# zouyuoz/SVS-UNet-PyTorch

Measured on AMD Instinct MI355X. Metric: spectrogram-tiles/sec (512x128) U-Net fwd+bwd (L1 train step incl. Adam), higher is better.
Workload: dtype f32; 1 GPU; train.py L1-loss step, 512x128 tiles, batch 64 per GPU; global_batch=64, parallelism=dp1, mode=train

## Files before the change

svs_unet_pytorch_amd/csrc/common.h:

```cpp
#pragma once
#include <hip/hip_runtime.h>
#include <stdint.h>
#include <stdio.h>
#include <string>

#include "../../include/svs_hip.h"

typedef float f32x4 __attribute__((ext_vector_type(4)));

void svs_set_error(const char* fmt, ...);

#define SVS_REQUIRE(cond, ...)                 \
  do {                                         \
    if (!(cond)) {                             \
      svs_set_error(__VA_ARGS__);              \
      return SVS_ERR_INVALID;                  \
    }                                          \
  } while (0)

#define SVS_CHECK_LAUNCH(name)                                                     \
  do {                                                                             \
    hipError_t e_ = hipGetLastError();                                             \
    if (e_ != hipSuccess) {                                                        \
      svs_set_error("%s: launch failed: %s", name, hipGetErrorString(e_));         \
      return (int)e_;                                                              \
    }                                                                              \
  } while (0)

#define SVS_HIP(call)                                                              \
  do {                                                                             \
    hipError_t e_ = (call);                                                        \
    if (e_ != hipSuccess) {                                                        \
      svs_set_error("%s failed: %s", #call, hipGetErrorString(e_));                \
      return (int)e_;                                                              \
    }                                                                              \
  } while (0)

static inline bool svs_aligned16(const void* p) { return (((uintptr_t)p) & 15u) == 0; }
static inline int svs_cdiv(long a, long b) { return (int)((a + b - 1) / b); }
static inline size_t svs_align_up(size_t x, size_t a) { return (x + a - 1) / a * a; }

enum SvsTune {
  SVS_TUNE_CONV_CFG, SVS_TUNE_CONV_KSPLIT, SVS_TUNE_CONV_WINDOW, SVS_TUNE_CONV_SKIP, SVS_TUNE_SKIP_REDUCE,
  SVS_TUNE_WGRAD_CFG, SVS_TUNE_WGRAD_KSPLIT, SVS_TUNE_WGRAD_SKIP, SVS_TUNE_WGRAD_WINDOW, SVS_TUNE_TRAIN_UNFUSED,
  SVS_TUNE_TRAIN_ONE_STREAM, SVS_TUNE_MFMA_SPLIT, SVS_TUNE_CONV_C1_TILED, SVS_TUNE_BF16_CFG, SVS_TUNE_BF16_KSPLIT,
  SVS_TUNE_BN_INLINE, SVS_TUNE_CONV_GWINDOW, SVS_TUNE_COUNT
};
long svs_tune(int key);
static inline bool svs_tune_on(int key) { return svs_tune(key) >= 0; }
static inline bool svs_tune_flag(int key) { return svs_tune(key) > 0; }

static inline int svs_conv_out(int n) { return (n + 1) / 2; }

__device__ __forceinline__ float svs_wave_sum(float v) {
#pragma unroll
  for (int o = 32; o > 0; o >>= 1) v += __shfl_xor(v, o, 64);
  return v;
}

__host__ __device__ __forceinline__ uint32_t svs_mix32(uint32_t x) {
  x ^= x >> 16; x *= 0x7FEB352Du; x ^= x >> 15; x *= 0x846CA68Bu; x ^= x >> 16;
  return x;
}
__host__ __device__ __forceinline__ uint32_t svs_u32(uint32_t seed, uint64_t idx) {
  uint32_t lo = (uint32_t)idx, hi = (uint32_t)(idx >> 32);
  uint32_t s = svs_mix32(seed + 1u);
  uint32_t h = svs_mix32(hi + 0x85EBCA6Bu * s);
  return svs_mix32(lo + 0x9E3779B9u * h);
}
```

svs_unet_pytorch_amd/csrc/gemm_wgrad.hip:

```cpp
#include <stdlib.h>

#include "internal.h"
#include "mfma_split.h"

struct WgradArgs {
  const float* s; long lds; int Hs, Ws, Cs;
  const float* l; long ldl; int Hl, Wl, Cl;
  int B;
  float* slab;
  long pix_per_split;
  int ws_shift, hs_shift;
  int b_shift;
};

template <int T> __device__ __forceinline__ void load_vec(const float* p, float (&f)[T]);
template <> __device__ __forceinline__ void load_vec<4>(const float* p, float (&f)[4]) {
  const f32x4 v = *(const f32x4*)p; f[0] = v[0]; f[1] = v[1]; f[2] = v[2]; f[3] = v[3];
}
template <> __device__ __forceinline__ void load_vec<2>(const float* p, float (&f)[2]) {
  const float2 v = *(const float2*)p; f[0] = v.x; f[1] = v.y;
}
template <int T> __device__ __forceinline__ void store_vec(float* p, const float (&f)[T]);
template <> __device__ __forceinline__ void store_vec<4>(float* p, const float (&f)[4]) { *(f32x4*)p = (f32x4){f[0], f[1], f[2], f[3]}; }
template <> __device__ __forceinline__ void store_vec<2>(float* p, const float (&f)[2]) { *(float2*)p = make_float2(f[0], f[1]); }
// ... 300 lines not shown
    }
  };
  auto stage = [&]() {
#pragma unroll
    for (int r = 0; r < RS; ++r) {
      const int e = t + 256 * r;
      if (e < NS) *(f32x4*)(&Ssm[(e / (CSB / 4)) * LS + (e % (CSB / 4)) * 4]) = sreg[r];
    }
#pragma unroll
    for (int r = 0; r < RL; ++r) {
      const int e = t + 256 * r;
      if (e < NL) *(f32x4*)(&Lsm[(e >> 2) * LL + (e & 3) * 4]) = lreg[r];
    }
  };

  f32x4 acc[25];
#pragma unroll
  for (int i = 0; i < 25; ++i) acc[i] = (f32x4){0.f, 0.f, 0.f, 0.f};
  const float* abase = &Ssm[(half * (TH / KS) * TW + q) * LS + mt * 16 + lrow];
  const float* bbase = &Lsm[(half * (TH / KS) * 2 * LW + 2 * q) * LL + lrow];

  if (tile_lo < tile_hi) fetch(tile_lo);
  for (int tile = tile_lo; tile < tile_hi; ++tile) {
    __syncthreads();
    stage();
    __syncthreads();
    if (tile + 1 < tile_hi) fetch(tile + 1);
#pragma unroll
    for (int ks = 0; ks < KSTEPS; ++ks) {
      const int sh = ks / 4, sg = ks % 4;
      const float a = abase[(sh * TW + sg * 4) * LS];
#pragma unroll
      for (int tap = 0; tap < 25; ++tap) {
        const int kh = tap / 5, kw = tap % 5;
        const float bv = bbase[((2 * sh + kh) * LW + 8 * sg + kw) * LL];
        acc[tap] = __builtin_amdgcn_mfma_f32_16x16x4f32(a, bv, acc[tap], 0, 0, 0);
      }
    }
  }
  const int Ntot = 25 * p.Cl;
  float* slab = p.slab + ((long)blockIdx.x * KS + half) * p.Cs * Ntot;
#pragma unroll
  for (int tap = 0; tap < 25; ++tap)
#pragma unroll
    for (int r = 0; r < 4; ++r)
      slab[(long)(m0 + mt * 16 + 4 * q + r) * Ntot + tap * p.Cl + cl0 + lrow] = acc[tap][r];
}

__global__ __launch_bounds__(256) void wgrad_reduce_kernel(const float* __restrict__ slab, int ksplit, int Cs, int Cl,
                                                           float* __restrict__ dw) {
  __shared__ float tile[25][65];
  const int clt = Cl < 64 ? Cl : 64;
  const int cs = blockIdx.x, cl0 = blockIdx.y * clt;
  const long zstride = (long)Cs * Cl * 25;
  const float* src0 = slab + (long)cs * 25 * Cl + cl0;
  const int q4 = clt >> 2;
  for (int e = threadIdx.x; e < 25 * q4; e += 256) {
    const int tap = e / q4, cl = (e - tap * q4) * 4;
    const float* src = src0 + (long)tap * Cl + cl;
    f32x4 acc = {0.f, 0.f, 0.f, 0.f};
    int z = 0;
    for (; z + 4 <= ksplit; z += 4, src += 4 * zstride) {
      const f32x4 a = *(const f32x4*)src, b = *(const f32x4*)(src + zstride), c = *(const f32x4*)(src + 2 * zstride), d = *(const f32x4*)(src + 3 * zstride);
      acc += a; acc += b; acc += c; acc += d;
    }
    for (; z < ksplit; ++z, src += zstride) acc += *(const f32x4*)src;
    tile[tap][cl] = acc[0]; tile[tap][cl + 1] = acc[1]; tile[tap][cl + 2] = acc[2]; tile[tap][cl + 3] = acc[3];
  }
  __syncthreads();
  float* dst = dw + ((long)cs * Cl + cl0) * 25;
  for (int e = threadIdx.x; e < 25 * clt; e += 256) {
    const int cl = e / 25, tap = e - cl * 25;
    dst[e] = tile[tap][cl];
  }
}

struct WgradTile { int cfg, BM, BN, ksplit; long pps; };
static WgradTile plan_wgrad(int B, int Hs, int Ws, int Cs, int Cl) {
  WgradTile pl{};
  if (Cs % 128 == 0) { pl.cfg = 0; pl.BM = 128; }
  else if (Cs % 64 == 0) { pl.cfg = 1; pl.BM = 64; }
  else { pl.cfg = 2; pl.BM = 32; }
  if (pl.cfg == 0 && ((long)B * Hs * Ws <= 1024 || Cl <= 32)) { pl.cfg = 1; pl.BM = 64; }
  if (svs_tune_on(SVS_TUNE_WGRAD_CFG)) {
    const int c = (int)svs_tune(SVS_TUNE_WGRAD_CFG);
    if (c == 0 && Cs % 128 == 0) { pl.cfg = 0; pl.BM = 128; }
    if (c == 1 && Cs % 64 == 0) { pl.cfg = 1; pl.BM = 64; }
    if (c == 2 && Cs % 32 == 0) { pl.cfg = 2; pl.BM = 32; }
  }
  pl.BN = 128;
  const long P = (long)B * Hs * Ws;
  const long blocks_mn = (long)(Cs / pl.BM) * ((25L * Cl + pl.BN - 1) / pl.BN);
  long ks = (1024 + blocks_mn - 1) / blocks_mn;
  const long cap = P / 128 > 1 ? P / 128 : 1;
  if (ks > cap) ks = cap;
  if (ks > 512) ks = 512;
  if (ks < 1) ks = 1;
  if (svs_tune_on(SVS_TUNE_WGRAD_KSPLIT)) { long f = svs_tune(SVS_TUNE_WGRAD_KSPLIT); if (f >= 1 && f <= cap) ks = f; }
  long pps = (P + ks - 1) / ks;
  pps = (pps + 15) / 16 * 16;
  ks = (P + pps - 1) / pps;
  pl.ksplit = (int)ks;
  pl.pps = pps;
  return pl;
}

#define WG_GROUPS 8

struct WgWinPlan { int eligible, use, MT, gy, gx, tpb, ntiles, nslab; };
static WgWinPlan plan_wgrad_window(int B, int Hs, int Ws, int Cs, int Cl) {
  WgWinPlan w{};
  w.eligible = (Cl == 16 || Cl == 32) && (Cs == 32 || Cs == 64 || Cs == 128);
  w.ntiles = B * ((Hs + 3) / 4) * ((Ws + 15) / 16);
  w.use = w.eligible && w.ntiles >= 1024;
  if (svs_tune_on(SVS_TUNE_WGRAD_WINDOW)) { const int f = (int)svs_tune(SVS_TUNE_WGRAD_WINDOW); w.use = (f == 0) ? 0 : (f == 2) ? w.eligible : w.use; }
  if (!w.eligible) return w;
  w.MT = (Cs % 64 == 0) ? 4 : 2;
  w.gy = (Cs / (16 * w.MT)) * (Cl / 16);
  int gx = 512 / w.gy;
  if (gx > w.ntiles) gx = w.ntiles;
  w.tpb = (w.ntiles + gx - 1) / gx;
  w.gx = (w.ntiles + w.tpb - 1) / w.tpb;
  w.nslab = w.gx * (4 / w.MT);
  return w;
}

struct WgradPlan {
  WgWinPlan win;
  WgradTile tile;
  int WM, WN, pf;
  bool skip, split;
  dim3 grid;
  int nslab;
};
static WgradPlan plan_wgrad_call(int B, int Hs, int Ws, int Cs, int Cl, long lds, int Hl, int Wl, long ldl) {
  WgradPlan p{};
  p.win = plan_wgrad_window(B, Hs, Ws, Cs, Cl);
  p.win.use = p.win.use && (long)Hs * Ws * lds * 4 < (1L << 31) && (long)Hl * Wl * ldl * 4 < (1L << 31);
  if (p.win.use) {
    p.grid = dim3(p.win.gx, p.win.gy);
    p.nslab = p.win.nslab;
    return p;
  }
  p.tile = plan_wgrad(B, Hs, Ws, Cs, Cl);
  p.WM = p.tile.cfg == 0 ? 2 : 1;
  p.WN = 4 / p.WM;
  const bool can_skip = B >= 16 && (B & (B - 1)) == 0 && (Ws & (Ws - 1)) == 0 && (long)B * Hs * Ws * lds * 4 < (1L << 31);
  const long f = svs_tune(SVS_TUNE_WGRAD_SKIP);
  p.skip = f == 0 ? false : f == 2 ? can_skip : can_skip && Ws <= 8;
  p.pf = p.skip && p.tile.cfg <= 1 ? 2 : 1;
  p.split = svs_tune(SVS_TUNE_MFMA_SPLIT) > 0;
  p.grid = dim3((unsigned)(Cs / p.tile.BM), (unsigned)((25 * Cl + p.tile.BN - 1) / p.tile.BN), (unsigned)p.tile.ksplit);
  p.nslab = p.tile.ksplit;
  return p;
}

size_t svs_wgrad_gemm_workspace(int B, int Hs, int Ws, int Cs, int Cl) {
  const WgWinPlan w = plan_wgrad_window(B, Hs, Ws, Cs, Cl);
  int nslab = plan_wgrad(B, Hs, Ws, Cs, Cl).ksplit;
  if (w.eligible && w.nslab > nslab) nslab = w.nslab;
  return ((size_t)nslab + WG_GROUPS) * Cs * 25 * Cl * sizeof(float);
}

static int wgrad_reduce_run(const float* slabs, int nslab, int Cs, int Cl, float* dw, float* tmp, hipStream_t stream) {
  const long n = (long)Cs * 25 * Cl;
  if (nslab > 2 * WG_GROUPS) {
    const int per = (nslab + WG_GROUPS - 1) / WG_GROUPS;
    const int groups = (nslab + per - 1) / per;
    if (int rc = svs_reduce_slabs_run(slabs, nslab, per, groups, n, tmp, stream)) return rc;
    slabs = tmp;
    nslab = groups;
  }
// ... 67 lines not shown
```

svs_unet_pytorch_amd/csrc/internal.h:

```cpp
#pragma once
#include "common.h"

enum { SVS_MODE_GATHER = 0, SVS_MODE_PARITY = 1 };

int svs_conv_gemm_run(int mode, const float* x, long ldx, int B, int H, int W, int C, const float* wp,
                      const float* bias, const float* scale, const float* shift, float slope, float* y, long ldy,
                      int Ho, int Wo, int N, int accumulate, void* ws, size_t ws_bytes, hipStream_t stream,
                      const char* who, float* stats = nullptr, int stats_cap = 0, int* stats_nblk = nullptr);
int svs_bn_finalize_run(const void* partial, int nblk, long P, int C, float eps, float momentum, float* running_mean,
                        float* running_var, long long* nbt, float* save_mean, float* save_invstd, hipStream_t stream);
int svs_bn_fin_act_apply_run(const void* partial, int rows, const float* raw, long ldr, long P, int C, long pixels_per_sample,
                             const float* gamma, const float* beta, float eps, float momentum, float* running_mean,
                             float* running_var, long long* nbt, float* save_mean, float* save_invstd, float slope,
                             const float* drop, float* y, long ldy, hipStream_t stream);
struct SvsSumJobs { int njobs; const float* partial[12]; int nblk[12]; int C[12]; float* out[12]; };
int svs_channel_sum_finalize_multi_run(const SvsSumJobs& jobs, hipStream_t stream);
size_t svs_bn_partial_floats(long P, int C);
int svs_bn_partial_rows(long P, int C);
size_t svs_conv_gemm_workspace(int mode, int B, int H, int W, int C, int Ho, int Wo, int N);

int svs_wgrad_gemm_run(const float* s, long lds, int B, int Hs, int Ws, int Cs, const float* l, long ldl, int Hl,
                       int Wl, int Cl, float* dw, void* ws, size_t ws_bytes, hipStream_t stream, const char* who);
size_t svs_wgrad_gemm_workspace(int B, int Hs, int Ws, int Cs, int Cl);

int svs_conv_c1_run(const float* x, int B, int H, int W, const float* w, const float* bias, const float* scale,
                    const float* shift, float slope, float* y, long ldy, int N, int accumulate, hipStream_t stream,
                    const char* who, long half = 0);
int svs_deconv_to1_run(const float* x, long ldx, int B, int H, int W, int C, const float* w, const float* bias,
                       float* y, int Ho, int Wo, int apply_sigmoid, hipStream_t stream, const char* who, long half = 0);
int svs_wgrad_c1_run(const float* s, long lds, int B, int Hs, int Ws, int Cs, const float* l, int Hl, int Wl,
                     float* dw, void* ws, size_t ws_bytes, hipStream_t stream, const char* who, long half = 0);
size_t svs_wgrad_c1_workspace(int B, int Hs, int Ws, int Cs);

int svs_channel_sum_run(const float* x, long ldx, long P, int C, float* out, void* ws, size_t ws_bytes, hipStream_t stream);
int svs_sum_run(const float* x, long n, float* out, void* ws, size_t ws_bytes, hipStream_t stream);
int svs_sigmoid_bwd_run(const float* mask, const float* dmask, long n, float* d_logit, hipStream_t stream);

int svs_reduce_slabs_run(const float* slab, int nslab, int per, int groups, long n, float* out, hipStream_t stream);

struct SvsPackJob { const float* w; float* wp; int N, C, kind, first_block; };
struct SvsPackJobs { SvsPackJob j[20]; int n; };
int svs_pack_all_run(SvsPackJobs& jobs, hipStream_t stream);

int svs_bn_bwd_run(const float* dy, long lddy, const float* raw, long ldr, long P, int C, long pixels_per_sample,
                   const float* gamma, const float* beta, const float* save_mean, const float* save_invstd, float slope,
                   const float* drop, float* d_raw, float* dgamma, float* dbeta, float* dbias, void* ws, size_t ws_bytes,
                   hipStream_t stream, float* dbias_partial = nullptr, SvsSumJobs* defer = nullptr);

int svs_fft_twiddles(int n, hipStream_t stream, const float2** out);

int svs_conv_gemm_describe(int mode, int B, int H, int W, int C, int Ho, int Wo, int N, long ldx, char* buf, size_t n);
int svs_wgrad_gemm_describe(int B, int Hs, int Ws, int Cs, int Cl, char* buf, size_t n);
int svs_conv_bf16_describe(int mode, int B, int H, int W, int C, int Ho, int Wo, int N, char* buf, size_t n);
```

svs_unet_pytorch_amd/csrc/net.hip:

```cpp
#include <math.h>
#include <algorithm>
#include <atomic>
#include <mutex>
#include <stdarg.h>
#include <stdlib.h>
#include <string.h>

#include "unet_desc.h"

static thread_local char g_err[512] = "";
void svs_set_error(const char* fmt, ...) {
  va_list ap;
  va_start(ap, fmt);
  vsnprintf(g_err, sizeof(g_err), fmt, ap);
  va_end(ap);
}
extern "C" const char* svs_last_error_string(void) { return g_err; }

static const char* const TUNE_NAMES[SVS_TUNE_COUNT] = {
    "CONV_CFG", "CONV_KSPLIT", "CONV_WINDOW", "CONV_SKIP", "SKIP_REDUCE", "WGRAD_CFG", "WGRAD_KSPLIT", "WGRAD_SKIP",
    "WGRAD_WINDOW", "TRAIN_UNFUSED", "TRAIN_ONE_STREAM", "MFMA_SPLIT", "CONV_C1_TILED", "BF16_CFG", "BF16_KSPLIT", "BN_INLINE",
    "CONV_GWINDOW"};
static std::atomic<long> g_tune[SVS_TUNE_COUNT];
static std::once_flag g_tune_once;
static void tune_load_env() {
  for (int k = 0; k < SVS_TUNE_COUNT; ++k) {
    char name[64];
    snprintf(name, sizeof(name), "SVS_%s", TUNE_NAMES[k]);
    const char* e = getenv(name);
    g_tune[k].store(e ? (*e ? atol(e) : 1) : -1, std::memory_order_relaxed);
  }
}
long svs_tune(int key) {
  std::call_once(g_tune_once, tune_load_env);
  return (key >= 0 && key < SVS_TUNE_COUNT) ? g_tune[key].load(std::memory_order_relaxed) : -1;
}
extern "C" int svs_tuning_set(const char* name, long value) {
  std::call_once(g_tune_once, tune_load_env);
  SVS_REQUIRE(name, "svs_tuning_set: null name");
  if (!strcmp(name, "*")) {
    if (value == -1) tune_load_env();
    else for (int k = 0; k < SVS_TUNE_COUNT; ++k) g_tune[k].store(value, std::memory_order_relaxed);
    return SVS_OK;
  }
  for (int k = 0; k < SVS_TUNE_COUNT; ++k)
    if (!strcmp(name, TUNE_NAMES[k])) { g_tune[k].store(value, std::memory_order_relaxed); return SVS_OK; }
  svs_set_error("svs_tuning_set: unknown switch '%s'", name);
  return SVS_ERR_INVALID;
}
extern "C" int svs_version(void) { return SVS_ABI_VERSION; }

extern "C" size_t svs_enc_block_workspace_bytes(int B, int H, int W, int C, int N) {
  return svs_conv_gemm_workspace(SVS_MODE_GATHER, B, H, W, C, svs_conv_out(H), svs_conv_out(W), N);
}
extern "C" int svs_enc_block_fwd(const float* x, int64_t ldx, int B, int H, int W, int C, const float* wp,
                                 const float* bias, const float* scale, const float* shift, float slope, float* y,
                                 int64_t ldy, int N, int accumulate, void* ws, size_t ws_bytes, hipStream_t stream) {
  if (C == 1) {
    SVS_REQUIRE(ldx == 1, "svs_enc_block_fwd: single-channel input must be dense (ldx=1)");
    return svs_conv_c1_run(x, B, H, W, wp, bias, scale, shift, slope, y, ldy, N, accumulate, stream, "svs_enc_block_fwd");
  }
  return svs_conv_gemm_run(SVS_MODE_GATHER, x, ldx, B, H, W, C, wp, bias, scale, shift, slope, y, ldy, svs_conv_out(H),
                           svs_conv_out(W), N, accumulate, ws, ws_bytes, stream, "svs_enc_block_fwd");
}
extern "C" size_t svs_dec_block_workspace_bytes(int B, int H, int W, int C, int Ho, int Wo, int N) {
  return svs_conv_gemm_workspace(SVS_MODE_PARITY, B, H, W, C, Ho, Wo, N);
}
extern "C" int svs_dec_block_fwd(const float* x, int64_t ldx, int B, int H, int W, int C, const float* wp,
                                 const float* bias, const float* scale, const float* shift, float slope, float* y,
                                 int64_t ldy, int Ho, int Wo, int N, int accumulate, void* ws, size_t ws_bytes,
                                 hipStream_t stream) {
  return svs_conv_gemm_run(SVS_MODE_PARITY, x, ldx, B, H, W, C, wp, bias, scale, shift, slope, y, ldy, Ho, Wo, N,
                           accumulate, ws, ws_bytes, stream, "svs_dec_block_fwd");
}
extern "C" int svs_out_block_fwd(const float* x, int64_t ldx, int B, int H, int W, int C, const float* w,
                                 const float* bias, float* y, int Ho, int Wo, int apply_sigmoid, hipStream_t stream) {
  return svs_deconv_to1_run(x, ldx, B, H, W, C, w, bias, y, Ho, Wo, apply_sigmoid, stream, "svs_out_block_fwd");
}
extern "C" int svs_enc_block_bwd_data(const float* dy, int64_t lddy, int B, int Ho, int Wo, int N, const float* wpar,
                                      float* dx, int64_t lddx, int H, int W, int C, int accumulate, void* ws,
                                      size_t ws_bytes, hipStream_t stream) {
  return svs_conv_gemm_run(SVS_MODE_PARITY, dy, lddy, B, Ho, Wo, N, wpar, nullptr, nullptr, nullptr, 0.f, dx, lddx, H, W,
                           C, accumulate, ws, ws_bytes, stream, "svs_enc_block_bwd_data");
}
extern "C" int svs_dec_block_bwd_data(const float* dy, int64_t lddy, int B, int Ho, int Wo, int N, const float* wgat,
                                      float* dx, int64_t lddx, int H, int W, int C, int accumulate, void* ws,
                                      size_t ws_bytes, hipStream_t stream) {
  if (N == 1) {
    SVS_REQUIRE(lddy == 1, "svs_dec_block_bwd_data: single-channel gradient must be dense");
    SVS_REQUIRE(H == svs_conv_out(Ho) && W == svs_conv_out(Wo), "svs_dec_block_bwd_data: geometry mismatch");
    return svs_conv_c1_run(dy, B, Ho, Wo, wgat, nullptr, nullptr, nullptr, 0.f, dx, lddx, C, accumulate, stream,
                           "svs_dec_block_bwd_data");
  }
  return svs_conv_gemm_run(SVS_MODE_GATHER, dy, lddy, B, Ho, Wo, N, wgat, nullptr, nullptr, nullptr, 0.f, dx, lddx, H, W,
                           C, accumulate, ws, ws_bytes, stream, "svs_dec_block_bwd_data");
}
extern "C" size_t svs_block_bwd_weight_workspace_bytes(int B, int Hs, int Ws, int Cs, int Cl) {
  size_t a = (Cl == 1) ? svs_wgrad_c1_workspace(B, Hs, Ws, Cs) : svs_wgrad_gemm_workspace(B, Hs, Ws, Cs, Cl);
  size_t b = svs_bn_workspace_bytes((int64_t)B * Hs * Ws * 4, Cs > Cl ? Cs : Cl);
  return a > b ? a : b;
}
extern "C" int svs_enc_block_bwd_weight(const float* dy, int64_t lddy, int B, int Ho, int Wo, int N, const float* x,
                                        int64_t ldx, int H, int W, int C, float* dw, float* db, void* ws,
                                        size_t ws_bytes, hipStream_t stream) {
  int rc;
// ... 321 lines not shown
  const float* dp = drop;
  for (int l = 6; l <= 10; ++l) {
    const Layer& D = LAYERS[l];
    const float* x = (l == 6) ? t.c6 : t.cat[D.lin];
    int stat_rows = 0;
    rc = svs_conv_gemm_run(SVS_MODE_PARITY, x, D.C, B, g.h[D.lin], g.w[D.lin], D.C, t.wfwd[l], v.b[l], nullptr, nullptr, 0.f,
                           t.raw[l], D.N, g.h[D.lout], g.w[D.lout], D.N, 0, t.scratch, t.scratch_bytes, stream,
                           "deconv forward", t.bnws, fused_rows, &stat_rows);
    if (rc) return rc;
    if ((rc = train_bn_act(c, l, stat_rows, bn_buffers, nbt, 0.f, dp, cat_half(t.cat, g, D.lout, 0), stream))) return rc;
    if (dp) dp += (long)B * D.N;
  }
  return svs_deconv_to1_run(t.cat[1], CH[1], B, g.h[1], g.w[1], LAYERS[11].C, v.w[11], v.b[11], mask, g.h[0], g.w[0], 1, stream,
                            "svs_unet_train_forward", level1_plane(g));
}

static int train_backward_impl(const TrainCall& c, float* grads, const float* mix, const float* drop, hipStream_t stream, int parts = 15) {
  const Geo& g = c.g; const TrainWs& t = c.t; const ParamView& v = c.v;
  const int B = g.B;
  int rc;
  auto G = [&](int idx) { return grads + svs_unet_param_offset(idx); };
  SvsSumJobs sums{};
  const bool unfused = svs_tune_flag(SVS_TUNE_TRAIN_UNFUSED);
  SideStream* sd = svs_tune_flag(SVS_TUNE_TRAIN_ONE_STREAM) ? nullptr : side_stream(stream);
  std::unique_lock<std::mutex> guard;
  if (sd) guard = std::unique_lock<std::mutex>(sd->mu);
  const hipStream_t wstream = sd ? sd->s : stream;
  float* const wscratch = sd ? t.scratch2 : t.scratch;
  const size_t wscratch_bytes = sd ? t.scratch2_bytes : t.scratch_bytes;
  int nfork_local = 0;
  int& nfork = sd ? sd->nfork : nfork_local;
  if (parts & 1) nfork = 0;
  auto layer_draw = [&](int l) -> float* { return sd ? t.d_raw_l[l] : t.d_raw; };
  auto fork = [&]() -> int {
    if (!sd) return SVS_OK;
    SVS_HIP(hipEventRecord(sd->fork[nfork & 3], stream));
    SVS_HIP(hipStreamWaitEvent(sd->s, sd->fork[nfork & 3], 0));
    return SVS_OK;
  };
  auto forked = [&]() -> int { ++nfork; return SVS_OK; };
  auto join = [&]() -> int {
    if (sd && nfork > 0) {
      SVS_HIP(hipEventRecord(sd->done[0], sd->s));
      SVS_HIP(hipStreamWaitEvent(stream, sd->done[0], 0));
    }
    return SVS_OK;
  };
  if (parts & 1) {
  const long half1 = level1_plane(g);
  if ((rc = fork())) return rc;
  if ((rc = svs_wgrad_c1_run(t.cat[1], CH[1], B, g.h[1], g.w[1], LAYERS[11].C, t.d_logit, g.h[0], g.w[0], G(44), wscratch, wscratch_bytes, wstream,
                             "deconv6 bwd_weight", half1))) return rc;
  if ((rc = svs_sum_run(t.d_logit, g.P[0], G(45), wscratch, wscratch_bytes, wstream))) return rc;
  if ((rc = forked())) return rc;
  if ((rc = svs_conv_c1_run(t.d_logit, B, g.h[0], g.w[0], v.w[11], nullptr, nullptr, nullptr, 0.f, t.dcat[1], CH[1], LAYERS[11].C, 0, stream,
                            "deconv6 bwd_data", half1))) return rc;
  long drop_off[11];
  { long o = 0; for (int l = 6; l <= 10; ++l) { drop_off[l] = o; o += (long)B * LAYERS[l].N; } }
  for (int l = 10; l >= 6; --l) {
    const int lin = LAYERS[l].lin, lout = LAYERS[l].lout, N = LAYERS[l].N, C = LAYERS[l].C;
    const float* x = (l == 6) ? t.c6 : t.cat[lin];
    const View dyv = cat_half(t.dcat, g, lout, 0);
    float* const d_raw = layer_draw(l);
    rc = svs_bn_bwd_run(dyv.p, dyv.ld, t.raw[l], N, g.P[lout], N, (long)g.h[lout] * g.w[lout], v.gamma[l], v.beta[l],
                        t.mean[l], t.invstd[l], 0.f, drop ? drop + drop_off[l] : nullptr, d_raw, G(4 * l + 2), G(4 * l + 3),
                        G(4 * l + 1), t.bnws, t.bnws_bytes, stream, unfused ? nullptr : t.dbias_part[l], &sums);
    if (rc) return rc;
    if ((rc = fork())) return rc;
    if ((rc = svs_dec_block_bwd_weight(x, C, B, g.h[lin], g.w[lin], C, d_raw, N, g.h[lout], g.w[lout], N, G(4 * l), nullptr,
                                       wscratch, wscratch_bytes, wstream))) return rc;
    if ((rc = forked())) return rc;
    float* dx = (l == 6) ? t.dc6 : t.dcat[lin];
    if ((rc = svs_dec_block_bwd_data(d_raw, N, B, g.h[lout], g.w[lout], N, t.wbwd[l], dx, C, g.h[lin], g.w[lin], C, 0,
                                     t.scratch, t.scratch_bytes, stream))) return rc;
  }
  if ((rc = svs_channel_sum_finalize_multi_run(sums, stream))) return rc;
  sums.njobs = 0;
  }
  if (!(parts & 14)) return SVS_OK;
  for (int k = 6; k >= 1; --k) {
    if (!(parts & (k == 6 ? 2 : k >= 4 ? 4 : 8))) continue;
    const int l = k - 1, N = CH[k], C = CH[k - 1];
    const View dyv = (k == 6) ? View{t.dc6, CH[6]} : cat_half(t.dcat, g, k, 1);
    float* const d_raw = layer_draw(l);
    rc = svs_bn_bwd_run(dyv.p, dyv.ld, t.raw[l], N, g.P[k], N, (long)g.h[k] * g.w[k], v.gamma[l], v.beta[l], t.mean[l], t.invstd[l],
                        LEAKY, nullptr, d_raw, G(4 * l + 2), G(4 * l + 3), G(4 * l + 1), t.bnws, t.bnws_bytes, stream,
                        unfused ? nullptr : t.dbias_part[l], &sums);
    if (rc) return rc;
    const View xi = (k == 1) ? View{const_cast<float*>(mix), 1} : cat_half(t.cat, g, k - 1, 1);
    const float* x = xi.p; const long ldx = xi.ld;
    if (k == 1) {
      if ((rc = svs_enc_block_bwd_weight(d_raw, N, B, g.h[k], g.w[k], N, x, ldx, g.h[k - 1], g.w[k - 1], C, G(4 * l), nullptr,
                                         t.scratch, t.scratch_bytes, stream))) return rc;
      continue;
    }
    if ((rc = fork())) return rc;
    if ((rc = svs_enc_block_bwd_weight(d_raw, N, B, g.h[k], g.w[k], N, x, ldx, g.h[k - 1], g.w[k - 1], C, G(4 * l), nullptr,
                                       wscratch, wscratch_bytes, wstream))) return rc;
    if ((rc = forked())) return rc;
    if (k >= 2) {
      const View dxs = cat_half(t.dcat, g, k - 1, 1);
      if ((rc = svs_enc_block_bwd_data(d_raw, N, B, g.h[k], g.w[k], N, t.wbwd[l], dxs.p, dxs.ld, g.h[k - 1], g.w[k - 1], C, 1,
                                       t.scratch, t.scratch_bytes, stream))) return rc;
    }
  }
  if ((rc = svs_channel_sum_finalize_multi_run(sums, stream))) return rc;
  return (parts & 8) ? join() : SVS_OK;
}

extern "C" int svs_unet_train_bwd_sync(hipStream_t consumer) {
  SideStream* sd = svs_tune_flag(SVS_TUNE_TRAIN_ONE_STREAM) ? nullptr : side_stream(consumer);
  if (!sd) return SVS_OK;
  std::lock_guard<std::mutex> guard(sd->mu);
  SVS_HIP(hipEventRecord(sd->sync, sd->s));
  SVS_HIP(hipStreamWaitEvent(consumer, sd->sync, 0));
  return SVS_OK;
}

extern "C" int svs_unet_train_forward(const float* params, float* bn_buffers, int64_t* num_batches_tracked, const float* mix,
                                      const float* drop, int B, int H, int W, float* mask, void* ws, size_t ws_bytes,
                                      hipStream_t stream) {
  SVS_REQUIRE(params && mix && mask && svs_aligned16(params) && svs_aligned16(mix) && svs_aligned16(mask), "svs_unet_train_forward: bad pointers");
  TrainCall c;
  const int rc = train_prologue("svs_unet_train_forward", params, B, H, W, ws, ws_bytes, c);
  if (rc) return rc;
  return train_forward_impl(c, bn_buffers, num_batches_tracked, mix, drop, mask, stream);
}

extern "C" int svs_unet_train_backward(const float* params, float* grads, const float* mix, const float* mask,
                                       const float* d_mask, const float* drop, int B, int H, int W, void* ws,
                                       size_t ws_bytes, hipStream_t stream) {
  SVS_REQUIRE(params && grads && mix && mask && d_mask && svs_aligned16(grads), "svs_unet_train_backward: bad pointers");
  TrainCall c;
  int rc = train_prologue("svs_unet_train_backward", params, B, H, W, ws, ws_bytes, c);
  if (rc) return rc;
  if ((rc = svs_sigmoid_bwd_run(mask, d_mask, c.g.P[0], c.t.d_logit, stream))) return rc;
  return train_backward_impl(c, grads, mix, drop, stream);
}

static int train_fwd_loss_impl(const TrainCall& c, float* bn_buffers, int64_t* nbt, const float* mix, const float* voc, const float* drop,
                               float loss_scale, float* mask, float* loss, hipStream_t stream) {
  float* m = mask ? mask : c.t.mask;
  const int rc = train_forward_impl(c, bn_buffers, nbt, mix, drop, m, stream);
  if (rc) return rc;
  return svs_l1_mask_loss_fwd_bwd(m, mix, voc, c.g.P[0], loss_scale, c.t.d_logit, loss, c.t.bnws, c.t.bnws_bytes, stream);
}

extern "C" int svs_unet_train_fwd_bwd(const float* params, float* grads, float* bn_buffers, int64_t* num_batches_tracked,
                                      const float* mix, const float* voc, const float* drop, int B, int H, int W,
                                      float loss_scale, float* mask, float* loss, void* ws, size_t ws_bytes,
                                      hipStream_t stream) {
  SVS_REQUIRE(params && grads && mix && voc && loss && svs_aligned16(params) && svs_aligned16(grads) && svs_aligned16(mix),
              "svs_unet_train_fwd_bwd: bad pointers");
  TrainCall c;
  int rc = train_prologue("svs_unet_train_fwd_bwd", params, B, H, W, ws, ws_bytes, c);
  if (rc) return rc;
  if ((rc = train_fwd_loss_impl(c, bn_buffers, num_batches_tracked, mix, voc, drop, loss_scale, mask, loss, stream))) return rc;
  return train_backward_impl(c, grads, mix, drop, stream);
}

extern "C" int svs_unet_train_fwd_loss(const float* params, float* bn_buffers, int64_t* num_batches_tracked, const float* mix,
                                       const float* voc, const float* drop, int B, int H, int W, float loss_scale, float* mask,
                                       float* loss, void* ws, size_t ws_bytes, hipStream_t stream) {
  SVS_REQUIRE(params && mix && voc && loss && svs_aligned16(params) && svs_aligned16(mix), "svs_unet_train_fwd_loss: bad pointers");
  TrainCall c;
  const int rc = train_prologue("svs_unet_train_fwd_loss", params, B, H, W, ws, ws_bytes, c);
// ... 53 lines not shown
```

svs_unet_pytorch_amd/csrc/special.hip:

```cpp
#include "internal.h"

struct C1Args {
  const float* x; int B, H, W;
  const float* w;
  const float* bias; const float* scale; const float* shift; float slope;
  float* y; long ldy; int Ho, Wo; int accumulate;
  long half;
};

__device__ __forceinline__ long chan_off(long pix, long ld, int sub, int subs_per_half, long half) {
  return pix * ld + (half ? (sub >= subs_per_half ? half + (sub - subs_per_half) * 4 : sub * 4) : sub * 4);
}

template <int COUT>
__global__ __launch_bounds__(256) void conv_c1_kernel(C1Args p) {
  constexpr int G = COUT / 4;
  constexpr int LD = COUT + 4;
  __shared__ __attribute__((aligned(16))) float tile[256 * LD];
  const float* __restrict__ w = p.w;
  const long P = (long)p.B * p.Ho * p.Wo;
  const long pix0 = (long)blockIdx.x * 256;
  const long pix = pix0 + threadIdx.x;
  if (pix < P) {
    const unsigned upix = (unsigned)pix, utmp = upix / (unsigned)p.Wo;
// ... 435 lines not shown
#pragma unroll
        for (int r = 0; r < 4; ++r) out[(i * 16 + 4 * q + r) * 25 + tap] = acc[i][nt][r];
      }
    }
}

__global__ __launch_bounds__(256) void reduce_slabs_kernel(const float* __restrict__ slab, int nslab, int per, long n,
                                                           float* __restrict__ out) {
  const long i = ((long)blockIdx.x * 256 + threadIdx.x) * 4;
  if (i >= n) return;
  const int z0 = blockIdx.y * per;
  int z1 = z0 + per;
  if (z1 > nslab) z1 = nslab;
  const float* src = slab + (long)z0 * n + i;
  f32x4 s = {0.f, 0.f, 0.f, 0.f};
  int z = z0;
  for (; z + 4 <= z1; z += 4, src += 4 * n) {
    const f32x4 a = *(const f32x4*)src, b = *(const f32x4*)(src + n), c = *(const f32x4*)(src + 2 * n), d = *(const f32x4*)(src + 3 * n);
    s += a; s += b; s += c; s += d;
  }
  for (; z < z1; ++z, src += n) s += *(const f32x4*)src;
  *(f32x4*)(out + (long)blockIdx.y * n + i) = s;
}

int svs_reduce_slabs_run(const float* slab, int nslab, int per, int groups, long n, float* out, hipStream_t stream) {
  hipLaunchKernelGGL(reduce_slabs_kernel, dim3((unsigned)((n / 4 + 255) / 256), (unsigned)groups), dim3(256), 0, stream, slab, nslab, per, n, out);
  SVS_CHECK_LAUNCH("reduce_slabs");
  return SVS_OK;
}

#define C1_GROUPS 32

static int wgrad_c1_blocks(long P) {
  long nb = (P + 2047) / 2048;
  if (nb > 1024) nb = 1024;
  if (nb < 1) nb = 1;
  return (int)nb;
}

size_t svs_wgrad_c1_workspace(int B, int Hs, int Ws, int Cs) {
  (void)B; (void)Hs; (void)Ws;
  return (size_t)(1024 + C1_GROUPS) * 25 * Cs * sizeof(float);
}

int svs_wgrad_c1_run(const float* s, long lds, int B, int Hs, int Ws, int Cs, const float* l, int Hl, int Wl,
                     float* dw, void* ws, size_t ws_bytes, hipStream_t stream, const char* who, long half) {
  SVS_REQUIRE(s && l && dw, "%s: null pointer", who);
  SVS_REQUIRE(Cs == 16 || Cs == 32, "%s: supports Cs=16/32, got %d", who, Cs);
  SVS_REQUIRE(Hs == svs_conv_out(Hl) && Ws == svs_conv_out(Wl), "%s: grid mismatch", who);
  SVS_REQUIRE(lds >= (half ? Cs / 2 : Cs) && lds % 4 == 0 && svs_aligned16(s), "%s: bad view", who);
  const long P = (long)B * Hs * Ws;
  const int nb = wgrad_c1_blocks(P);
  const size_t need = svs_wgrad_c1_workspace(B, Hs, Ws, Cs);
  if (!ws || ws_bytes < need) {
    svs_set_error("%s: workspace too small (%zu < %zu)", who, ws_bytes, need);
    return SVS_ERR_WORKSPACE;
  }
  WgC1Args a{s, lds, B, Hs, Ws, l, Hl, Wl, (float*)ws, (P + nb - 1) / nb, half};
  int nslab = nb;
  const int ntiles = B * ((Hs + 3) / 4) * ((Ws + 15) / 16);
  if (ntiles >= 256) {
    int waves = ntiles < 1024 ? ntiles : 1024;
    waves = (waves + 3) / 4 * 4;
    if (waves > 1024) waves = 1024;
    const int tpw = (ntiles + waves - 1) / waves;
    waves = ((ntiles + tpw - 1) / tpw + 3) / 4 * 4;
    nslab = waves;
    if (Cs == 16) hipLaunchKernelGGL(wgrad_c1_mfma_kernel<16>, dim3(waves / 4), dim3(256), 0, stream, a, ntiles, tpw);
    else hipLaunchKernelGGL(wgrad_c1_mfma_kernel<32>, dim3(waves / 4), dim3(256), 0, stream, a, ntiles, tpw);
  } else if (Cs == 16) hipLaunchKernelGGL(wgrad_c1_kernel<16>, dim3(nb), dim3(256), 0, stream, a);
  else hipLaunchKernelGGL(wgrad_c1_kernel<32>, dim3(nb), dim3(256), 0, stream, a);
  SVS_CHECK_LAUNCH("wgrad_c1");
  const long n = 25L * Cs;
  float* tmp = (float*)ws + (size_t)nslab * n;
  const int groups = nslab < C1_GROUPS ? nslab : C1_GROUPS;
  const int per = (nslab + groups - 1) / groups;
  const unsigned gx = (unsigned)((n / 4 + 255) / 256);
  hipLaunchKernelGGL(reduce_slabs_kernel, dim3(gx, (unsigned)groups), dim3(256), 0, stream, (const float*)ws, nslab, per, n, tmp);
  SVS_CHECK_LAUNCH("reduce_slabs");
  hipLaunchKernelGGL(reduce_slabs_kernel, dim3(gx, 1), dim3(256), 0, stream, (const float*)tmp, groups, groups, n, dw);
  SVS_CHECK_LAUNCH("reduce_slabs");
  return SVS_OK;
}
```

Baseline: 19070 tiles/s.

## Fuse first-layer BN/LeakyReLU backward with conv1 weight gradient in one kernel

Adds a fused kernel for the first encoder layer (16 output channels, 1 input channel). It recomputes the activation-gradient masking and normalized input on the fly, accumulates the BN reduction sums, and computes the weight-gradient GEMM with MFMA from staged input patches. The BN correction is then applied algebraically in a double-precision finalize kernel. This avoids materialising d_raw and the separate BN-backward, channel-sum and wgrad passes, at the cost of a custom reduction path and a new workspace layout. It also removes the WGRAD_CFG tune knob, which shifts the tune enum indices.

Result: no change. 19070 tiles/s, median of 2 (+0.0%).

```diff
diff --git a/svs_unet_pytorch_amd/csrc/common.h b/svs_unet_pytorch_amd/csrc/common.h
--- a/svs_unet_pytorch_amd/csrc/common.h
+++ b/svs_unet_pytorch_amd/csrc/common.h
@@ -42,9 +42,9 @@
 
 enum SvsTune {
   SVS_TUNE_CONV_CFG, SVS_TUNE_CONV_KSPLIT, SVS_TUNE_CONV_WINDOW, SVS_TUNE_CONV_SKIP, SVS_TUNE_SKIP_REDUCE,
-  SVS_TUNE_WGRAD_CFG, SVS_TUNE_WGRAD_KSPLIT, SVS_TUNE_WGRAD_SKIP, SVS_TUNE_WGRAD_WINDOW, SVS_TUNE_TRAIN_UNFUSED,
+  SVS_TUNE_WGRAD_KSPLIT, SVS_TUNE_WGRAD_SKIP, SVS_TUNE_WGRAD_WINDOW, SVS_TUNE_TRAIN_UNFUSED,
   SVS_TUNE_TRAIN_ONE_STREAM, SVS_TUNE_MFMA_SPLIT, SVS_TUNE_CONV_C1_TILED, SVS_TUNE_BF16_CFG, SVS_TUNE_BF16_KSPLIT,
-  SVS_TUNE_BN_INLINE, SVS_TUNE_CONV_GWINDOW, SVS_TUNE_COUNT
+  SVS_TUNE_BN_INLINE, SVS_TUNE_CONV_GWINDOW, SVS_TUNE_C1_BWD_FUSED, SVS_TUNE_COUNT
 };
 long svs_tune(int key);
 static inline bool svs_tune_on(int key) { return svs_tune(key) >= 0; }
diff --git a/svs_unet_pytorch_amd/csrc/gemm_wgrad.hip b/svs_unet_pytorch_amd/csrc/gemm_wgrad.hip
--- a/svs_unet_pytorch_amd/csrc/gemm_wgrad.hip
+++ b/svs_unet_pytorch_amd/csrc/gemm_wgrad.hip
@@ -406,12 +406,6 @@
   else if (Cs % 64 == 0) { pl.cfg = 1; pl.BM = 64; }
   else { pl.cfg = 2; pl.BM = 32; }
   if (pl.cfg == 0 && ((long)B * Hs * Ws <= 1024 || Cl <= 32)) { pl.cfg = 1; pl.BM = 64; }
-  if (svs_tune_on(SVS_TUNE_WGRAD_CFG)) {
-    const int c = (int)svs_tune(SVS_TUNE_WGRAD_CFG);
-    if (c == 0 && Cs % 128 == 0) { pl.cfg = 0; pl.BM = 128; }
-    if (c == 1 && Cs % 64 == 0) { pl.cfg = 1; pl.BM = 64; }
-    if (c == 2 && Cs % 32 == 0) { pl.cfg = 2; pl.BM = 32; }
-  }
   pl.BN = 128;
   const long P = (long)B * Hs * Ws;
   const long blocks_mn = (long)(Cs / pl.BM) * ((25L * Cl + pl.BN - 1) / pl.BN);
diff --git a/svs_unet_pytorch_amd/csrc/internal.h b/svs_unet_pytorch_amd/csrc/internal.h
--- a/svs_unet_pytorch_amd/csrc/internal.h
+++ b/svs_unet_pytorch_amd/csrc/internal.h
@@ -31,6 +31,9 @@
 int svs_wgrad_c1_run(const float* s, long lds, int B, int Hs, int Ws, int Cs, const float* l, int Hl, int Wl,
                      float* dw, void* ws, size_t ws_bytes, hipStream_t stream, const char* who, long half = 0);
 size_t svs_wgrad_c1_workspace(int B, int Hs, int Ws, int Cs);
+int svs_conv1_bwd_fused_run(const float* raw, long ldr, const float* dy, long lddy, int B, int Hs, int Ws, const float* l, int Hl,
+                            int Wl, const float* gamma, const float* beta, const float* mean, const float* invstd, float slope,
+                            float* dw, float* dbias, float* dgamma, float* dbeta, void* ws, size_t ws_bytes, hipStream_t stream);
 
 int svs_channel_sum_run(const float* x, long ldx, long P, int C, float* out, void* ws, size_t ws_bytes, hipStream_t stream);
 int svs_sum_run(const float* x, long n, float* out, void* ws, size_t ws_bytes, hipStream_t stream);
diff --git a/svs_unet_pytorch_amd/csrc/net.hip b/svs_unet_pytorch_amd/csrc/net.hip
--- a/svs_unet_pytorch_amd/csrc/net.hip
+++ b/svs_unet_pytorch_amd/csrc/net.hip
@@ -18,9 +18,9 @@
 extern "C" const char* svs_last_error_string(void) { return g_err; }
 
 static const char* const TUNE_NAMES[SVS_TUNE_COUNT] = {
-    "CONV_CFG", "CONV_KSPLIT", "CONV_WINDOW", "CONV_SKIP", "SKIP_REDUCE", "WGRAD_CFG", "WGRAD_KSPLIT", "WGRAD_SKIP",
+    "CONV_CFG", "CONV_KSPLIT", "CONV_WINDOW", "CONV_SKIP", "SKIP_REDUCE", "WGRAD_KSPLIT", "WGRAD_SKIP",
     "WGRAD_WINDOW", "TRAIN_UNFUSED", "TRAIN_ONE_STREAM", "MFMA_SPLIT", "CONV_C1_TILED", "BF16_CFG", "BF16_KSPLIT", "BN_INLINE",
-    "CONV_GWINDOW"};
+    "CONV_GWINDOW", "C1_BWD_FUSED"};
 static std::atomic<long> g_tune[SVS_TUNE_COUNT];
 static std::once_flag g_tune_once;
 static void tune_load_env() {
@@ -508,6 +508,11 @@
     if (!(parts & (k == 6 ? 2 : k >= 4 ? 4 : 8))) continue;
     const int l = k - 1, N = CH[k], C = CH[k - 1];
     const View dyv = (k == 6) ? View{t.dc6, CH[6]} : cat_half(t.dcat, g, k, 1);
+    if (k == 1 && svs_tune(SVS_TUNE_C1_BWD_FUSED) != 0) {
+      if ((rc = svs_conv1_bwd_fused_run(t.raw[0], N, dyv.p, dyv.ld, B, g.h[1], g.w[1], mix, g.h[0], g.w[0], v.gamma[0], v.beta[0],
+                                        t.mean[0], t.invstd[0], LEAKY, G(0), G(1), G(2), G(3), t.scratch, t.scratch_bytes, stream))) return rc;
+      continue;
+    }
     float* const d_raw = layer_draw(l);
     rc = svs_bn_bwd_run(dyv.p, dyv.ld, t.raw[l], N, g.P[k], N, (long)g.h[k] * g.w[k], v.gamma[l], v.beta[l], t.mean[l], t.invstd[l],
                         LEAKY, nullptr, d_raw, G(4 * l + 2), G(4 * l + 3), G(4 * l + 1), t.bnws, t.bnws_bytes, stream,
diff --git a/svs_unet_pytorch_amd/csrc/special.hip b/svs_unet_pytorch_amd/csrc/special.hip
--- a/svs_unet_pytorch_amd/csrc/special.hip
+++ b/svs_unet_pytorch_amd/csrc/special.hip
@@ -541,3 +541,203 @@
   SVS_CHECK_LAUNCH("reduce_slabs");
   return SVS_OK;
 }
+
+enum { C1F_M = 800, C1F_S1 = 828, C1F_SX = 844, C1F_S2 = 860, C1F_N = 876 };
+
+struct C1BwdArgs {
+  const float* raw; long ldr; const float* dy; long lddy; int B, Hs, Ws;
+  const float* l; int Hl, Wl;
+  const float* gamma; const float* beta; const float* mean; const float* invstd; float slope;
+  float* slab;
+};
+
+__global__ __launch_bounds__(256) void conv1_bwd_fused_kernel(C1BwdArgs p, int ntiles, int nwaves) {
+  constexpr int TH = 4, TW = 16, LS = 48;
+  constexpr int LH = 2 * TH + 3, LW = 2 * TW + 3, LWP = LW + 1;
+  constexpr int NLP = (LH * LW + 63) / 64;
+  __shared__ __attribute__((aligned(16))) float Ssm[4][TH * TW * LS];
+  __shared__ float Lsm[4][LH * LWP];
+  const int t = threadIdx.x, lane = t & 63, wave = t >> 6;
+  const int lrow = lane & 15, q = lane >> 4;
+  const int c4 = lane & 3, pcol = lane >> 2;
+  float* const sS = Ssm[wave];
+  float* const sL = Lsm[wave];
+  const int tiles_w = (p.Ws + TW - 1) / TW, tiles_h = (p.Hs + TH - 1) / TH;
+  const int gw = blockIdx.x * 4 + wave;
+  const int tile_lo = (int)((long)gw * ntiles / nwaves), tile_hi = (int)((long)(gw + 1) * ntiles / nwaves);
+
+  const f32x4 mean4 = *(const f32x4*)(p.mean + c4 * 4), inv4 = *(const f32x4*)(p.invstd + c4 * 4);
+  const f32x4 k4 = *(const f32x4*)(p.gamma + c4 * 4) * inv4, beta4 = *(const f32x4*)(p.beta + c4 * 4);
+  f32x4 xreg[TH], greg[TH];
+  float lreg[NLP];
+  int vbits = 0;
+  auto fetch = [&](int tile) {
+    const int tw0 = (tile % tiles_w) * TW, th0 = ((tile / tiles_w) % tiles_h) * TH;
+    const long b = tile / (tiles_w * tiles_h);
+    vbits = 0;
+#pragma unroll
+    for (int r = 0; r < TH; ++r) {
+      const int sh = th0 + r, sw = tw0 + pcol;
+      f32x4 x = {0.f, 0.f, 0.f, 0.f}, g = x;
+      if (sh < p.Hs && sw < p.Ws) {
+        const long pix = (b * p.Hs + sh) * p.Ws + sw;
+        x = *(const f32x4*)(p.raw + pix * p.ldr + c4 * 4);
+        g = *(const f32x4*)(p.dy + pix * p.lddy + c4 * 4);
+        vbits |= 1 << r;
+      }
+      xreg[r] = x; greg[r] = g;
+    }
+    const float* img = p.l + b * p.Hl * p.Wl;
+#pragma unroll
+    for (int r = 0; r < NLP; ++r) {
+      const int e = lane + 64 * r;
+      const int wr = e / LW, wc = e % LW;
+      const int ih = 2 * th0 - 2 + wr, iw = 2 * tw0 - 2 + wc;
+      float v = 0.f;
+      if (e < LH * LW && (unsigned)ih < (unsigned)p.Hl && (unsigned)iw < (unsigned)p.Wl) v = img[(long)ih * p.Wl + iw];
+      lreg[r] = v;
+    }
+  };
+  f32x4 s1 = {0.f, 0.f, 0.f, 0.f}, sx = s1, s2 = s1;
+  auto stage = [&]() {
+#pragma unroll
+    for (int r = 0; r < TH; ++r) {
+      const f32x4 xm = xreg[r] - mean4;
+      const f32x4 z = xm * k4 + beta4;
+      f32x4 dz = greg[r], xh = xm * inv4;
+#pragma unroll
+      for (int k = 0; k < 4; ++k) dz[k] = z[k] > 0.f ? dz[k] : dz[k] * p.slope;
+      if (!((vbits >> r) & 1)) xh = (f32x4){0.f, 0.f, 0.f, 0.f};
+      s1 += dz;
+      sx += xh;
+      s2 += dz * xh;
+      float* dst = &sS[(r * TW + pcol) * LS + c4 * 4];
+      *(f32x4*)dst = dz;
+      *(f32x4*)(dst + 16) = xh;
+    }
+#pragma unroll
+    for (int r = 0; r < NLP; ++r) {
+      const int e = lane + 64 * r;
+      if (e < LH * LW) sL[(e / LW) * LWP + e % LW] = lreg[r];
+    }
+  };
+  f32x4 acc[2][2];
+#pragma unroll
+  for (int i = 0; i < 2; ++i) { acc[i][0] = (f32x4){0.f, 0.f, 0.f, 0.f}; acc[i][1] = acc[i][0]; }
+  float msum[2] = {0.f, 0.f};
+  int boff[2];
+#pragma unroll
+  for (int nt = 0; nt < 2; ++nt) {
+    const int tap = min(nt * 16 + lrow, 24);
+    boff[nt] = (tap / 5) * LWP + tap % 5 + 2 * q;
+  }
+  if (tile_lo < tile_hi) fetch(tile_lo);
+  for (int tile = tile_lo; tile < tile_hi; ++tile) {
+    const int nc = p.Ws - (tile % tiles_w) * TW, nr = p.Hs - ((tile / tiles_w) % tiles_h) * TH;
+    stage();
+    __builtin_amdgcn_wave_barrier();
+    if (tile + 1 < tile_hi) fetch(tile + 1);
+#pragma unroll
+    for (int ks = 0; ks < TH * TW / 4; ++ks) {
+      const int sh = ks / 4, sg = ks % 4;
+      const bool inside = sh < nr && sg * 4 + q < nc;
+      float bv[2];
+#pragma unroll
+      for (int nt = 0; nt < 2; ++nt) {
+        bv[nt] = sL[boff[nt] + 2 * sh * LWP + 8 * sg];
+        msum[nt] += inside ? bv[nt] : 0.f;
+      }
+#pragma unroll
+      for (int i = 0; i < 2; ++i) {
+        const float a = sS[(sh * TW + sg * 4 + q) * LS + i * 16 + lrow];
+#pragma unroll
+        for (int nt = 0; nt < 2; ++nt) acc[i][nt] = __builtin_amdgcn_mfma_f32_16x16x4f32(a, bv[nt], acc[i][nt], 0, 0, 0);
+      }
+    }
+    __builtin_amdgcn_wave_barrier();
+  }
+  float* out = p.slab + (long)gw * C1F_N;
+#pragma unroll
+  for (int nt = 0; nt < 2; ++nt) {
+    const int tap = nt * 16 + lrow;
+    float m = msum[nt];
+    m += __shfl_xor(m, 16, 64);
+    m += __shfl_xor(m, 32, 64);
+    if (tap < 25) {
+#pragma unroll
+      for (int i = 0; i < 2; ++i)
+#pragma unroll
+        for (int r = 0; r < 4; ++r) out[(i * 16 + 4 * q + r) * 25 + tap] = acc[i][nt][r];
+      if (q == 0) out[C1F_M + tap] = m;
+    }
+  }
+  if (lane < 3) out[C1F_M + 25 + lane] = 0.f;
+#pragma unroll
+  for (int k = 0; k < 4; ++k) {
+    float a = s1[k], b = sx[k], c = s2[k];
+#pragma unroll
+    for (int o = 4; o < 64; o <<= 1) { a += __shfl_xor(a, o, 64); b += __shfl_xor(b, o, 64); c += __shfl_xor(c, o, 64); }
+    if (lane < 4) { out[C1F_S1 + lane * 4 + k] = a; out[C1F_SX + lane * 4 + k] = b; out[C1F_S2 + lane * 4 + k] = c; }
+  }
+}
+
+__global__ __launch_bounds__(256) void conv1_bwd_finalize_kernel(const float* __restrict__ grp, int groups, long P,
+                                                                 const float* __restrict__ gamma, const float* __restrict__ invstd,
+                                                                 float* dw, float* dbias, float* dgamma, float* dbeta) {
+  __shared__ double tot[C1F_N];
+  const int t = threadIdx.x;
+  for (int i = t; i < C1F_N; i += 256) {
+    double s = 0.0;
+    for (int g = 0; g < groups; ++g) s += (double)grp[(long)g * C1F_N + i];
+    tot[i] = s;
+  }
+  __syncthreads();
+  for (int i = t; i < 400; i += 256) {
+    const int c = i / 25, tap = i - c * 25;
+    const double k = (double)gamma[c] * (double)invstd[c];
+    const double m1 = tot[C1F_S1 + c] / (double)P, m2 = tot[C1F_S2 + c] / (double)P;
+    dw[i] = (float)(k * (tot[i] - m1 * tot[C1F_M + tap] - m2 * tot[400 + i]));
+  }
+  if (t < 16) {
+    const double k = (double)gamma[t] * (double)invstd[t];
+    const double a = tot[C1F_S1 + t], b = tot[C1F_S2 + t];
+    const double m1 = a / (double)P, m2 = b / (double)P;
+    dbeta[t] = (float)a;
+    dgamma[t] = (float)b;
+    dbias[t] = (float)(k * (a - (double)P * m1 - m2 * tot[C1F_SX + t]));
+  }
+}
+
+int svs_conv1_bwd_fused_run(const float* raw, long ldr, const float* dy, long lddy, int B, int Hs, int Ws, const float* l, int Hl,
+                            int Wl, const float* gamma, const float* beta, const float* mean, const float* invstd, float slope,
+                            float* dw, float* dbias, float* dgamma, float* dbeta, void* ws, size_t ws_bytes, hipStream_t stream) {
+  const char* who = "svs_conv1_bwd_fused";
+  SVS_REQUIRE(raw && dy && l && gamma && beta && mean && invstd && dw && dbias && dgamma && dbeta, "%s: null pointer", who);
+  SVS_REQUIRE(B > 0 && Hs == svs_conv_out(Hl) && Ws == svs_conv_out(Wl), "%s: grid mismatch", who);
+  SVS_REQUIRE(ldr >= 16 && ldr % 4 == 0 && lddy >= 16 && lddy % 4 == 0 && svs_aligned16(raw) && svs_aligned16(dy), "%s: bad view", who);
+  SVS_REQUIRE(svs_aligned16(gamma) && svs_aligned16(beta) && svs_aligned16(mean) && svs_aligned16(invstd), "%s: unaligned statistics", who);
+  const long ntiles_l = (long)B * ((Hs + 3) / 4) * ((Ws + 15) / 16);
+  SVS_REQUIRE(ntiles_l < (1L << 31), "%s: too many tiles", who);
+  const int ntiles = (int)ntiles_l;
+  const size_t slab_bytes = C1F_N * sizeof(float);
+  long waves = ws ? (long)(ws_bytes / slab_bytes) - C1_GROUPS : 0;
+  if (waves > 1024) waves = 1024;
+  if (waves > (ntiles + 3) / 4 * 4) waves = (ntiles + 3) / 4 * 4;
+  waves = waves / 4 * 4;
+  if (waves < 4) {
+    svs_set_error("%s: workspace too small (%zu < %zu)", who, ws_bytes, (size_t)(4 + C1_GROUPS) * slab_bytes);
+    return SVS_ERR_WORKSPACE;
+  }
+  C1BwdArgs a{raw, ldr, dy, lddy, B, Hs, Ws, l, Hl, Wl, gamma, beta, mean, invstd, slope, (float*)ws};
+  hipLaunchKernelGGL(conv1_bwd_fused_kernel, dim3((unsigned)(waves / 4)), dim3(256), 0, stream, a, ntiles, (int)waves);
+  SVS_CHECK_LAUNCH("conv1_bwd_fused");
+  const int nslab = (int)waves;
+  float* tmp = (float*)ws + (size_t)nslab * C1F_N;
+  const int groups = nslab < C1_GROUPS ? nslab : C1_GROUPS;
+  const int per = (nslab + groups - 1) / groups;
+  if (int rc = svs_reduce_slabs_run((const float*)ws, nslab, per, groups, C1F_N, tmp, stream)) return rc;
+  hipLaunchKernelGGL(conv1_bwd_finalize_kernel, dim3(1), dim3(256), 0, stream, (const float*)tmp, groups, (long)B * Hs * Ws, gamma,
+                     invstd, dw, dbias, dgamma, dbeta);
+  SVS_CHECK_LAUNCH("conv1_bwd_finalize");
+  return SVS_OK;
+}
```
